# bacon205/Multimodal_eeg_fmri

Measured on AMD Instinct MI355X. Metric: pairs_per_sec_per_node, higher is better.
Workload: dtype bf16

## Files before the change

### multimodal_eeg_fmri_amd/csrc/attention.hip

```cpp
#include "common.h"

namespace {

constexpr int VR = 32;

__device__ __forceinline__ bf16x8 tr_frag32(const bf16* tile, int row0, int lane) {
    const int li = lane & 15, g = lane >> 4;
    const bf16* p = tile + (row0 + 8 * (g >> 1) + (li >> 2)) * VR + (g & 1) * 16 + 4 * (li & 3);
    typedef __attribute__((address_space(3))) s16x4 lds_s16x4;
    union { s16x4 s[2]; bf16x8 v; } u;
    u.s[0] = __builtin_amdgcn_ds_read_tr16_b64_v4i16((lds_s16x4*)(p));
    u.s[1] = __builtin_amdgcn_ds_read_tr16_b64_v4i16((lds_s16x4*)(p + 4 * VR));
    return u.v;
}

__device__ __forceinline__ int vperm(int key) {
    return (key & ~12) | ((key & 4) << 1) | ((key & 8) >> 1);
}

__device__ __forceinline__ uint32_t attn_block_hash(uint32_t seed, int bh, int q, int key, int L) {
    const uint32_t Lh = ((uint32_t)L + 1u) >> 1;
    uint32_t x = (((uint32_t)bh * Lh + ((uint32_t)q >> 1)) * Lh + ((uint32_t)key >> 1)) * 0x9E3779B1u + seed;
    x ^= x >> 13;
    x = __umul24(x, 0xB5297Bu);
    x ^= x >> 15;
    return x;
}
template <bool ALONG_KEYS>
__device__ __forceinline__ void attn_keep2(uint32_t seed, int bh, int mine, int other, int L, uint32_t thresh8, bool& k0, bool& k1) {
    if (ALONG_KEYS) {
        const uint32_t x = attn_block_hash(seed, bh, mine, other, L) >> (16 * (mine & 1));
        k0 = (x & 0xFFu) >= thresh8;
        k1 = ((x >> 8) & 0xFFu) >= thresh8;
    } else {
        const uint32_t x = attn_block_hash(seed, bh, other, mine, L) >> (8 * (mine & 1));
        k0 = (x & 0xFFu) >= thresh8;
        k1 = ((x >> 16) & 0xFFu) >= thresh8;
    }
}

__device__ __forceinline__ float xhalf_max(float v) {
    const auto r = __builtin_amdgcn_permlane32_swap(__float_as_uint(v), __float_as_uint(v), false, false);
    return fmaxf(__uint_as_float(r[0]), __uint_as_float(r[1]));
}
__device__ __forceinline__ float xhalf_sum(float v) {
    const auto r = __builtin_amdgcn_permlane32_swap(__float_as_uint(v), __float_as_uint(v), false, false);
    return __uint_as_float(r[0]) + __uint_as_float(r[1]);
}

__device__ __forceinline__ float fast_exp2(float x) { return __builtin_amdgcn_exp2f(x); }

__device__ __forceinline__ void zero8(bf16x8& v) {
#pragma unroll
    for (int j = 0; j < 8; ++j) v[j] = (bf16)0.f;
}

constexpr int KCH = 128;
constexpr int QCH = 128;

template <int DHP>
struct Hd {
    static_assert(DHP == 32 || DHP == 64, "padded head width");
    static constexpr int NS = DHP / 16;
    static constexpr int NT = DHP / 32;
    static constexpr int KS = DHP + 8;
    static constexpr int NG = DHP / 8;
    static __device__ __forceinline__ int tr_off(int rows, int row, int sg) { return (sg >> 2) * rows * VR + row * VR + (sg & 3) * 8; }
};

template <int DHP, bool EXACT>
struct Dims {
    int L, H, dh_;
    Dims(int L, int H, int dh) : L(L), H(H), dh_(dh) {}
    __device__ int dh() const { return dh_; }
};
template <int DHP>
struct Dims<DHP, true> {
    int L, H;
    Dims(int L, int H, int) : L(L), H(H) {}
    __device__ constexpr int dh() const { return DHP; }
};

template <int DHP, bool EXACT, bool DROP, bool FULL, bool MASK>
__global__ __launch_bounds__(256) void attn_fwd_kernel(const bf16* __restrict__ qkv, bf16* __restrict__ out,
                                                       float* __restrict__ lse, const Dims<DHP, EXACT> dm, float scale_log2,
                                                       uint32_t dthresh, uint32_t dseed, float dinv,
                                                       const uint32_t* epoch, const float* __restrict__ amask, size_t amask_bh) {
    using T = Hd<DHP>;
    constexpr int NS = T::NS, NT = T::NT, KS = T::KS, NG = T::NG;
    const int L = dm.L, H = dm.H, dh = dm.dh();
    dseed = mm_eff_seed(dseed, epoch);
    if (MASK) amask += (size_t)(blockIdx.z * H + blockIdx.y) * amask_bh;
    __shared__ __attribute__((aligned(16))) bf16 Ks[KCH * KS];
    __shared__ __attribute__((aligned(16))) bf16 Vs[NT * KCH * VR];
    const int E = H * dh, E3 = 3 * E;
    const int b = blockIdx.z, h = blockIdx.y;
    const int tid = threadIdx.x, lane = tid & 63, wave = tid >> 6;
    const int lr = lane & 31, lh = lane >> 5;
    const int q = blockIdx.x * 128 + wave * 32 + lr;
    const bf16* base = qkv + (size_t)b * L * E3 + h * dh;

    bf16x8 qf[NS];
#pragma unroll
    for (int s = 0; s < NS; ++s) {
        zero8(qf[s]);
        if (q < L && 16 * s + 8 * lh < dh) qf[s] = *reinterpret_cast<const bf16x8*>(base + (size_t)q * E3 + 16 * s + 8 * lh);
    }
    f32x16 o[NT];
#pragma unroll
    for (int t = 0; t < NT; ++t)
#pragma unroll
        for (int r = 0; r < 16; ++r) o[t][r] = 0.f;
    float m_run = -INFINITY, l_run = 0.f;

    constexpr int NI = KCH * NG / 256;
    uint4 kreg[NI], vreg[NI];
    auto load_chunk = [&](int k0) __attribute__((always_inline)) {
        const int kn = min(KCH, L - k0);
#pragma unroll
        for (int i = 0; i < NI; ++i) {
            const int s = tid + i * 256, key = s / NG, sg = s % NG;
            kreg[i] = make_uint4(0, 0, 0, 0); vreg[i] = make_uint4(0, 0, 0, 0);
            if (key < kn && sg * 8 < dh) {
                const bf16* row = base + (size_t)(k0 + key) * E3;
                kreg[i] = *reinterpret_cast<const uint4*>(row + E + sg * 8);
                vreg[i] = *reinterpret_cast<const uint4*>(row + 2 * E + sg * 8);
            }
        }
    };
    load_chunk(0);
#pragma unroll
    for (int s = 0; s < NS; ++s) asm volatile("" : : "v"(qf[s]));
    for (int k0 = 0; k0 < L; k0 += KCH) {
        const int kn = min(KCH, L - k0);
        const int kn32 = (kn + 31) & ~31;
        __syncthreads();
#pragma unroll
        for (int i = 0; i < NI; ++i) {
            const int s = tid + i * 256, key = s / NG, sg = s % NG;
            if (key >= kn32) continue;
            *reinterpret_cast<uint4*>(Ks + key * KS + sg * 8) = kreg[i];
            *reinterpret_cast<uint4*>(Vs + T::tr_off(KCH, vperm(key), sg)) = vreg[i];
        }
        __syncthreads();
        if (k0 + KCH < L) load_chunk(k0 + KCH);
        bf16x8 kfr[NS];
#pragma unroll
        for (int s = 0; s < NS; ++s) kfr[s] = *reinterpret_cast<const bf16x8*>(Ks + lr * KS + 16 * s + 8 * lh);
        for (int kt = 0; kt < kn32; kt += 32) {
            f32x16 sacc;
#pragma unroll
            for (int r = 0; r < 16; ++r) sacc[r] = 0.f;
#pragma unroll
            for (int s = 0; s < NS; ++s) sacc = __builtin_amdgcn_mfma_f32_32x32x16_bf16(kfr[s], qf[s], sacc, 0, 0, 0);
            bf16x8 vfr[NT][2];
#pragma unroll
            for (int t = 0; t < NT; ++t)
#pragma unroll
                for (int s = 0; s < 2; ++s) vfr[t][s] = tr_frag32(Vs + t * KCH * VR, kt + 16 * s, lane);
            if (kt + 32 < kn32)
#pragma unroll
                for (int s = 0; s < NS; ++s) kfr[s] = *reinterpret_cast<const bf16x8*>(Ks + (kt + 32 + lr) * KS + 16 * s + 8 * lh);
            const float sc2 = MASK ? 1.f : scale_log2;
            float mx = -INFINITY;
#pragma unroll
            for (int r = 0; r < 16; ++r) {
                const int key = kt + (r & 3) + 8 * (r >> 2) + 4 * lh;
                float sc = sacc[r];
                if (MASK) {
                    sc *= scale_log2;
                    if (key < kn) sc += amask[(size_t)min(q, L - 1) * L + k0 + key] * 1.4426950408889634f;
                }
                sacc[r] = (FULL || key < kn) ? sc : -INFINITY;
                mx = fmaxf(mx, sacc[r]);
            }
            mx = xhalf_max(mx);
            if (__builtin_amdgcn_ballot_w64(mx * sc2 > m_run + 8.f)) {
                const float m_new = fmaxf(m_run, mx * sc2);
                const float alpha = fast_exp2(m_run - ((MASK && m_new == -INFINITY) ? 0.f : m_new));
                l_run *= alpha;
                m_run = m_new;
#pragma unroll
                for (int t = 0; t < NT; ++t)
#pragma unroll
                    for (int r = 0; r < 16; ++r) o[t][r] *= alpha;
            }
            const float m_neg = (MASK && m_run == -INFINITY) ? 0.f : -m_run;
            float ps = 0.f;
            union { bf16x8 v[2]; bf16x2 h[8]; } pu;
#pragma unroll
            for (int r = 0; r < 16; r += 2) {
                float p0 = fast_exp2(fmaf(sacc[r], sc2, m_neg)), p1 = fast_exp2(fmaf(sacc[r + 1], sc2, m_neg));
                ps += p0;
                ps += p1;
                if (DROP) {
                    bool kp0, kp1;
                    attn_keep2<true>(dseed, b * H + h, q, k0 + kt + (r & 3) + 8 * (r >> 2) + 4 * lh, L, dthresh, kp0, kp1);
                    p0 = kp0 ? p0 : 0.f; p1 = kp1 ? p1 : 0.f;
                }
                typedef __attribute__((ext_vector_type(2))) float f32x2_t;
                pu.h[r >> 1] = __builtin_convertvector((f32x2_t){p0, p1}, bf16x2);
            }
            l_run += ps;
#pragma unroll
            for (int t = 0; t < NT; ++t)
#pragma unroll
                for (int s = 0; s < 2; ++s) o[t] = __builtin_amdgcn_mfma_f32_32x32x16_bf16(vfr[t][s], pu.v[s], o[t], 0, 0, 0);
        }
    }
    const float l_tot = xhalf_sum(l_run);
    const float inv = (DROP ? dinv : 1.f) / l_tot;
    if (q < L) {
        bf16* orow = out + ((size_t)b * L + q) * E + h * dh;
#pragma unroll
        for (int t = 0; t < NT; ++t)
#pragma unroll
            for (int g = 0; g < 4; ++g) {
                const int d = 32 * t + 8 * g + 4 * lh;
                if (d >= dh) continue;
                bf16x4 v = {(bf16)(o[t][4 * g] * inv), (bf16)(o[t][4 * g + 1] * inv), (bf16)(o[t][4 * g + 2] * inv), (bf16)(o[t][4 * g + 3] * inv)};
                *reinterpret_cast<bf16x4*>(orow + d) = v;
            }
        if (lse && lh == 0) lse[((size_t)b * H + h) * L + q] = (m_run + log2f(l_tot)) * 0.6931471805599453f;
    }
}

template <int DHP, bool EXACT, bool DROP, bool FULL, bool MASK>
__global__ __launch_bounds__(256) void attn_bwd_dq_kernel(const bf16* __restrict__ qkv, const bf16* __restrict__ out,
                                                          const bf16* __restrict__ dout, const float* __restrict__ lse,
                                                          bf16* __restrict__ dqkv, float* __restrict__ delta,
                                                          const Dims<DHP, EXACT> dm, float scale, uint32_t dthresh,
                                                          uint32_t dseed, float dinv, const uint32_t* epoch,
                                                          const float* __restrict__ amask, size_t amask_bh) {
    using T = Hd<DHP>;
    constexpr int NS = T::NS, NT = T::NT, KS = T::KS, NG = T::NG;
    const int L = dm.L, H = dm.H, dh = dm.dh();
    dseed = mm_eff_seed(dseed, epoch);
    if (MASK) amask += (size_t)(blockIdx.z * H + blockIdx.y) * amask_bh;
    __shared__ __attribute__((aligned(16))) bf16 Ks[KCH * KS];
    __shared__ __attribute__((aligned(16))) bf16 Vs[KCH * KS];
    __shared__ __attribute__((aligned(16))) bf16 Kr[NT * KCH * VR];
    const int E = H * dh, E3 = 3 * E;
    const int b = blockIdx.z, h = blockIdx.y;
    const int tid = threadIdx.x, lane = tid & 63, wave = tid >> 6;
    const int lr = lane & 31, lh = lane >> 5;
    const int q = blockIdx.x * 128 + wave * 32 + lr;
    const bool qok = q < L;
    const bf16* base = qkv + (size_t)b * L * E3 + h * dh;
    const float scale_log2 = scale * 1.4426950408889634f;

    bf16x8 qf[NS], dof[NS];
    float dl = 0.f;
#pragma unroll
    for (int s = 0; s < NS; ++s) {
        zero8(qf[s]); zero8(dof[s]);
        if (qok && 16 * s + 8 * lh < dh) {
            qf[s] = *reinterpret_cast<const bf16x8*>(base + (size_t)q * E3 + 16 * s + 8 * lh);
            const size_t oi = ((size_t)b * L + q) * E + h * dh + 16 * s + 8 * lh;
            dof[s] = *reinterpret_cast<const bf16x8*>(dout + oi);
            const bf16x8 of = *reinterpret_cast<const bf16x8*>(out + oi);
#pragma unroll
            for (int j = 0; j < 8; ++j) dl += (float)dof[s][j] * (float)of[j];
        }
    }
    dl = xhalf_sum(dl);
    const float lse2 = qok ? lse[((size_t)b * H + h) * L + q] * 1.4426950408889634f : 0.f;
    if (qok && lh == 0) delta[((size_t)b * H + h) * L + q] = dl;

    f32x16 dq[NT];
#pragma unroll
    for (int t = 0; t < NT; ++t)
#pragma unroll
        for (int r = 0; r < 16; ++r) dq[t][r] = 0.f;

    constexpr int NI = KCH * NG / 256;
    uint4 kreg[NI], vreg[NI];
    auto load_chunk = [&](int k0) __attribute__((always_inline)) {
        const int kn = min(KCH, L - k0);
#pragma unroll
        for (int i = 0; i < NI; ++i) {
            const int s = tid + i * 256, key = s / NG, sg = s % NG;
            kreg[i] = make_uint4(0, 0, 0, 0); vreg[i] = make_uint4(0, 0, 0, 0);
            if (key < kn && sg * 8 < dh) {
                const bf16* row = base + (size_t)(k0 + key) * E3;
                kreg[i] = *reinterpret_cast<const uint4*>(row + E + sg * 8);
                vreg[i] = *reinterpret_cast<const uint4*>(row + 2 * E + sg * 8);
            }
        }
    };
    load_chunk(0);
#pragma unroll
    for (int s = 0; s < NS; ++s) asm volatile("" : : "v"(qf[s]), "v"(dof[s]));
    asm volatile("" : : "v"(dl), "v"(lse2));
    for (int k0 = 0; k0 < L; k0 += KCH) {
        const int kn = min(KCH, L - k0);
        const int kn32 = (kn + 31) & ~31;
        __syncthreads();
#pragma unroll
        for (int i = 0; i < NI; ++i) {
            const int s = tid + i * 256, key = s / NG, sg = s % NG;
            if (key >= kn32) continue;
            *reinterpret_cast<uint4*>(Ks + key * KS + sg * 8) = kreg[i];
            *reinterpret_cast<uint4*>(Vs + key * KS + sg * 8) = vreg[i];
            *reinterpret_cast<uint4*>(Kr + T::tr_off(KCH, vperm(key), sg)) = kreg[i];
        }
        __syncthreads();
        if (k0 + KCH < L) load_chunk(k0 + KCH);
        for (int kt = 0; kt < kn32; kt += 32) {
            f32x16 sacc, dp;
#pragma unroll
            for (int r = 0; r < 16; ++r) { sacc[r] = 0.f; dp[r] = 0.f; }
            bf16x8 kfr[NS], vfr[NS];
#pragma unroll
            for (int s = 0; s < NS; ++s) {
                kfr[s] = *reinterpret_cast<const bf16x8*>(Ks + (kt + lr) * KS + 16 * s + 8 * lh);
                vfr[s] = *reinterpret_cast<const bf16x8*>(Vs + (kt + lr) * KS + 16 * s + 8 * lh);
            }
#pragma unroll
            for (int s = 0; s < NS; ++s) {
                sacc = __builtin_amdgcn_mfma_f32_32x32x16_bf16(kfr[s], qf[s], sacc, 0, 0, 0);
                dp = __builtin_amdgcn_mfma_f32_32x32x16_bf16(vfr[s], dof[s], dp, 0, 0, 0);
            }
            bf16x8 ktfr[NT][2];
#pragma unroll
            for (int t = 0; t < NT; ++t)
#pragma unroll
                for (int s = 0; s < 2; ++s) ktfr[t][s] = tr_frag32(Kr + t * KCH * VR, kt + 16 * s, lane);
            bf16x8 dsf[2];
            bool kp[16];
            if (DROP)
#pragma unroll
                for (int r = 0; r < 16; r += 2)
                    attn_keep2<true>(dseed, b * H + h, q, k0 + kt + (r & 3) + 8 * (r >> 2) + 4 * lh, L, dthresh, kp[r], kp[r + 1]);
#pragma unroll
            for (int r = 0; r < 16; ++r) {
                const int key = kt + (r & 3) + 8 * (r >> 2) + 4 * lh;
                float sc = fmaf(sacc[r], scale_log2, -lse2);
                if (MASK && key < kn) sc += amask[(size_t)min(q, L - 1) * L + k0 + key] * 1.4426950408889634f;
                const float p = (FULL || key < kn) ? fast_exp2(sc) : 0.f;
                float dpr = dp[r];
                if (DROP) dpr = fmaf(kp[r] ? dpr : 0.f, dinv, -dl);
                else dpr -= dl;
                dsf[r >> 3][r & 7] = (bf16)(p * dpr);
            }
#pragma unroll
            for (int t = 0; t < NT; ++t)
#pragma unroll
                for (int s = 0; s < 2; ++s) dq[t] = __builtin_amdgcn_mfma_f32_32x32x16_bf16(ktfr[t][s], dsf[s], dq[t], 0, 0, 0);
        }
    }
    if (qok) {
        bf16* drow = dqkv + ((size_t)b * L + q) * E3 + h * dh;
#pragma unroll
        for (int t = 0; t < NT; ++t)
#pragma unroll
            for (int g = 0; g < 4; ++g) {
                const int d = 32 * t + 8 * g + 4 * lh;
                if (d >= dh) continue;
                bf16x4 v = {(bf16)(dq[t][4 * g] * scale), (bf16)(dq[t][4 * g + 1] * scale), (bf16)(dq[t][4 * g + 2] * scale), (bf16)(dq[t][4 * g + 3] * scale)};
                *reinterpret_cast<bf16x4*>(drow + d) = v;
            }
    }
}

template <int DHP, bool EXACT, bool DROP, bool FULL, bool MASK>
__global__ __launch_bounds__(256) void attn_bwd_dkv_kernel(const bf16* __restrict__ qkv, const bf16* __restrict__ dout,
                                                           const float* __restrict__ lse, const float* __restrict__ delta,
                                                           bf16* __restrict__ dqkv, const Dims<DHP, EXACT> dm, float scale,
                                                           uint32_t dthresh, uint32_t dseed, float dinv,
                                                           const uint32_t* epoch, const float* __restrict__ amask, size_t amask_bh) {
    using T = Hd<DHP>;
    constexpr int NS = T::NS, NT = T::NT, KS = T::KS, NG = T::NG;
    const int L = dm.L, H = dm.H, dh = dm.dh();
    dseed = mm_eff_seed(dseed, epoch);
    if (MASK) amask += (size_t)(blockIdx.z * H + blockIdx.y) * amask_bh;
    __shared__ __attribute__((aligned(16))) bf16 Qs[QCH * KS];
    __shared__ __attribute__((aligned(16))) bf16 Ds[QCH * KS];
    __shared__ __attribute__((aligned(16))) bf16 Qr[NT * QCH * VR];
    __shared__ __attribute__((aligned(16))) bf16 Dr[NT * QCH * VR];
    __shared__ float Ls[QCH], Dl[QCH];
    const int E = H * dh, E3 = 3 * E;
    const int b = blockIdx.z, h = blockIdx.y;
    const int tid = threadIdx.x, lane = tid & 63, wave = tid >> 6;
    const int lr = lane & 31, lh = lane >> 5;
    const int key = blockIdx.x * 128 + wave * 32 + lr;
    const bool kok = key < L;
    const bf16* base = qkv + (size_t)b * L * E3 + h * dh;
    const float scale_log2 = scale * 1.4426950408889634f;

    bf16x8 kf[NS], vf[NS];
#pragma unroll
    for (int s = 0; s < NS; ++s) {
        zero8(kf[s]); zero8(vf[s]);
        if (kok && 16 * s + 8 * lh < dh) {
            kf[s] = *reinterpret_cast<const bf16x8*>(base + (size_t)key * E3 + E + 16 * s + 8 * lh);
            vf[s] = *reinterpret_cast<const bf16x8*>(base + (size_t)key * E3 + 2 * E + 16 * s + 8 * lh);
        }
    }
    f32x16 dk[NT], dv[NT];
#pragma unroll
    for (int t = 0; t < NT; ++t)
#pragma unroll
        for (int r = 0; r < 16; ++r) { dk[t][r] = 0.f; dv[t][r] = 0.f; }

    constexpr int NI = QCH * NG / 256;
    static_assert(QCH <= 256, "one lse / delta value per thread");
    uint4 qreg[NI], dreg[NI];
    float lreg = INFINITY, dlreg = 0.f;
    auto load_chunk = [&](int q0) __attribute__((always_inline)) {
        const int qn = min(QCH, L - q0);
#pragma unroll
        for (int i = 0; i < NI; ++i) {
            const int s = tid + i * 256, qi = s / NG, sg = s % NG;
            qreg[i] = make_uint4(0, 0, 0, 0); dreg[i] = make_uint4(0, 0, 0, 0);
            if (qi < qn && sg * 8 < dh) {
                qreg[i] = *reinterpret_cast<const uint4*>(base + (size_t)(q0 + qi) * E3 + sg * 8);
                dreg[i] = *reinterpret_cast<const uint4*>(dout + ((size_t)b * L + q0 + qi) * E + h * dh + sg * 8);
            }
        }
        const bool ok = tid < qn;
        lreg = ok ? lse[((size_t)b * H + h) * L + q0 + tid] : INFINITY;
        dlreg = ok ? delta[((size_t)b * H + h) * L + q0 + tid] : 0.f;
    };
    load_chunk(0);
#pragma unroll
    for (int s = 0; s < NS; ++s) asm volatile("" : : "v"(kf[s]), "v"(vf[s]));
    for (int q0 = 0; q0 < L; q0 += QCH) {
        const int qn = min(QCH, L - q0);
        const int qn32 = (qn + 31) & ~31;
        __syncthreads();
#pragma unroll
        for (int i = 0; i < NI; ++i) {
            const int s = tid + i * 256, qi = s / NG, sg = s % NG;
            if (qi >= qn32) continue;
            *reinterpret_cast<uint4*>(Qs + qi * KS + sg * 8) = qreg[i];
            *reinterpret_cast<uint4*>(Ds + qi * KS + sg * 8) = dreg[i];
            *reinterpret_cast<uint4*>(Qr + T::tr_off(QCH, vperm(qi), sg)) = qreg[i];
            *reinterpret_cast<uint4*>(Dr + T::tr_off(QCH, vperm(qi), sg)) = dreg[i];
        }
        if (tid < qn32) { Ls[tid] = lreg * 1.4426950408889634f; Dl[tid] = dlreg; }
        __syncthreads();
        if (q0 + QCH < L) load_chunk(q0 + QCH);
        for (int qt = 0; qt < qn32; qt += 32) {
            f32x16 sacc, dp;
#pragma unroll
            for (int r = 0; r < 16; ++r) { sacc[r] = 0.f; dp[r] = 0.f; }
            bf16x8 qar[NS], dar[NS];
#pragma unroll
            for (int s = 0; s < NS; ++s) {
                qar[s] = *reinterpret_cast<const bf16x8*>(Qs + (qt + lr) * KS + 16 * s + 8 * lh);
                dar[s] = *reinterpret_cast<const bf16x8*>(Ds + (qt + lr) * KS + 16 * s + 8 * lh);
            }
#pragma unroll
            for (int s = 0; s < NS; ++s) {
                sacc = __builtin_amdgcn_mfma_f32_32x32x16_bf16(qar[s], kf[s], sacc, 0, 0, 0);
                dp = __builtin_amdgcn_mfma_f32_32x32x16_bf16(dar[s], vf[s], dp, 0, 0, 0);
            }
            bf16x8 dtar[NT][2], qtar[NT][2];
#pragma unroll
            for (int t = 0; t < NT; ++t)
#pragma unroll
                for (int s = 0; s < 2; ++s) {
                    dtar[t][s] = tr_frag32(Dr + t * QCH * VR, qt + 16 * s, lane);
                    qtar[t][s] = tr_frag32(Qr + t * QCH * VR, qt + 16 * s, lane);
                }
            bf16x8 pf[2], dsf[2];
            bool kp[16];
            if (DROP)
#pragma unroll
                for (int r = 0; r < 16; r += 2)
                    attn_keep2<false>(dseed, b * H + h, key, q0 + qt + (r & 3) + 8 * (r >> 2) + 4 * lh, L, dthresh, kp[r], kp[r + 1]);
#pragma unroll
            for (int r = 0; r < 16; ++r) {
                const int qi = qt + (r & 3) + 8 * (r >> 2) + 4 * lh;
                float sc = fmaf(sacc[r], scale_log2, -Ls[qi]);
                if (MASK && kok && qi < qn) sc += amask[(size_t)(q0 + qi) * L + key] * 1.4426950408889634f;
                const float p = (FULL || kok) ? fast_exp2(sc) : 0.f;
                pf[r >> 3][r & 7] = (bf16)((!DROP || kp[r]) ? p : 0.f);
                const float u = DROP ? fmaf(kp[r] ? dp[r] : 0.f, dinv, -Dl[qi]) : dp[r] - Dl[qi];
                dsf[r >> 3][r & 7] = (bf16)(p * u);
            }
#pragma unroll
            for (int t = 0; t < NT; ++t)
#pragma unroll
                for (int s = 0; s < 2; ++s) {
                    dv[t] = __builtin_amdgcn_mfma_f32_32x32x16_bf16(dtar[t][s], pf[s], dv[t], 0, 0, 0);
                    dk[t] = __builtin_amdgcn_mfma_f32_32x32x16_bf16(qtar[t][s], dsf[s], dk[t], 0, 0, 0);
                }
        }
    }
    if (kok) {
        bf16* krow = dqkv + ((size_t)b * L + key) * E3 + E + h * dh;
        bf16* vrow = krow + E;
        const float dvs = DROP ? dinv : 1.f;
#pragma unroll
        for (int t = 0; t < NT; ++t)
#pragma unroll
            for (int g = 0; g < 4; ++g) {
                const int d = 32 * t + 8 * g + 4 * lh;
                if (d >= dh) continue;
                bf16x4 a = {(bf16)(dk[t][4 * g] * scale), (bf16)(dk[t][4 * g + 1] * scale), (bf16)(dk[t][4 * g + 2] * scale), (bf16)(dk[t][4 * g + 3] * scale)};
                bf16x4 c = {(bf16)(dv[t][4 * g] * dvs), (bf16)(dv[t][4 * g + 1] * dvs), (bf16)(dv[t][4 * g + 2] * dvs), (bf16)(dv[t][4 * g + 3] * dvs)};
                *reinterpret_cast<bf16x4*>(krow + d) = a;
                *reinterpret_cast<bf16x4*>(vrow + d) = c;
            }
    }
}

uint32_t attn_thresh(float p) { return p > 0.f ? (uint32_t)((double)p * 256.0 + 0.5) : 0u; }
float attn_keep_scale(uint32_t t) { return t ? 256.f / (256.f - (float)t) : 1.f; }

bool hd_supported(int dh) { return dh >= 16 && dh <= 64 && dh % 8 == 0; }

template <int DHP, bool EXACT>
void launch_fwd(const void* qkv, void* out, float* lse, int B, int L, int H, int dh, float scale, float drop_p,
                uint32_t seed, const uint32_t* seed_epoch, const float* attn_mask, int per_head, hipStream_t st) {
    const uint32_t dth = attn_thresh(drop_p);
    const size_t mask_bh = attn_mask && per_head ? (size_t)L * L : 0;
    const bool full = L % KCH == 0;
    auto kern = dth ? (full ? attn_fwd_kernel<DHP, EXACT, true, true, false> : attn_fwd_kernel<DHP, EXACT, true, false, false>)
                    : (full ? attn_fwd_kernel<DHP, EXACT, false, true, false> : attn_fwd_kernel<DHP, EXACT, false, false, false>);
    if (attn_mask) kern = dth ? attn_fwd_kernel<DHP, EXACT, true, false, true> : attn_fwd_kernel<DHP, EXACT, false, false, true>;
    hipLaunchKernelGGL(kern, dim3(ceil_div(L, 128), H, B), dim3(256), 0, st, (const bf16*)qkv, (bf16*)out, lse,
                       Dims<DHP, EXACT>(L, H, dh), scale * 1.4426950408889634f, dth, seed, attn_keep_scale(dth), seed_epoch,
                       attn_mask, mask_bh);
}

template <int DHP, bool EXACT>
int launch_bwd(const void* qkv, const void* out, const void* dout, const float* lse, void* dqkv, float* delta_ws,
               int B, int L, int H, int dh, float scale, float drop_p, uint32_t seed, const uint32_t* seed_epoch,
               const float* attn_mask, int per_head, hipStream_t st) {
    const uint32_t dth = attn_thresh(drop_p);
    const float dinv = attn_keep_scale(dth);
    const size_t mask_bh = attn_mask && per_head ? (size_t)L * L : 0;
    const bool full = L % KCH == 0 && L % QCH == 0;
    auto kdq = dth ? (full ? attn_bwd_dq_kernel<DHP, EXACT, true, true, false> : attn_bwd_dq_kernel<DHP, EXACT, true, false, false>)
                   : (full ? attn_bwd_dq_kernel<DHP, EXACT, false, true, false> : attn_bwd_dq_kernel<DHP, EXACT, false, false, false>);
    auto kdkv = dth ? (full ? attn_bwd_dkv_kernel<DHP, EXACT, true, true, false> : attn_bwd_dkv_kernel<DHP, EXACT, true, false, false>)
                    : (full ? attn_bwd_dkv_kernel<DHP, EXACT, false, true, false> : attn_bwd_dkv_kernel<DHP, EXACT, false, false, false>);
    if (attn_mask) {
        kdq = dth ? attn_bwd_dq_kernel<DHP, EXACT, true, false, true> : attn_bwd_dq_kernel<DHP, EXACT, false, false, true>;
        kdkv = dth ? attn_bwd_dkv_kernel<DHP, EXACT, true, false, true> : attn_bwd_dkv_kernel<DHP, EXACT, false, false, true>;
    }
    const dim3 grid(ceil_div(L, 128), H, B);
    const Dims<DHP, EXACT> dm(L, H, dh);
    hipLaunchKernelGGL(kdq, grid, dim3(256), 0, st, (const bf16*)qkv, (const bf16*)out, (const bf16*)dout, lse,
                       (bf16*)dqkv, delta_ws, dm, scale, dth, seed, dinv, seed_epoch, attn_mask, mask_bh);
    int rc = mm_check_launch(EXACT ? "attn_bwd_dq" : "attn_bwd_hd_dq");
    if (rc) return rc;
    hipLaunchKernelGGL(kdkv, grid, dim3(256), 0, st, (const bf16*)qkv, (const bf16*)dout, lse, delta_ws, (bf16*)dqkv,
                       dm, scale, dth, seed, dinv, seed_epoch, attn_mask, mask_bh);
    return mm_check_launch(EXACT ? "attn_bwd_dkv" : "attn_bwd_hd_dkv");
}

}

extern "C" {

int mm_attn_fwd(const void* qkv, void* out, float* lse, int B, int L, int H, int head_dim, float scale,
                float drop_p, uint32_t seed, const uint32_t* seed_epoch, const float* attn_mask, int attn_mask_per_head,
                hipStream_t st) {
    MM_REQUIRE(drop_p >= 0.f && drop_p < 1.f, "attn_fwd: drop_p");
    MM_REQUIRE(qkv && out && B > 0 && L > 0 && H > 0, "attn_fwd: null/invalid");
    MM_REQUIRE(head_dim == 32, "attn_fwd: head_dim=%d (kernel is specialised for 32)", head_dim);
    launch_fwd<32, true>(qkv, out, lse, B, L, H, head_dim, scale, drop_p, seed, seed_epoch, attn_mask, attn_mask_per_head, st);
    return mm_check_launch("attn_fwd");
}

int mm_attn_bwd(const void* qkv, const void* out, const void* dout, const float* lse, void* dqkv, float* delta_ws,
                int B, int L, int H, int head_dim, float scale, float drop_p, uint32_t seed,
                const uint32_t* seed_epoch, const float* attn_mask, int attn_mask_per_head, hipStream_t st) {
    MM_REQUIRE(qkv && out && dout && lse && dqkv && delta_ws && B > 0 && L > 0 && H > 0, "attn_bwd: null/invalid");
    MM_REQUIRE(head_dim == 32, "attn_bwd: head_dim=%d (kernel is specialised for 32)", head_dim);
    return launch_bwd<32, true>(qkv, out, dout, lse, dqkv, delta_ws, B, L, H, head_dim, scale, drop_p, seed, seed_epoch,
                                attn_mask, attn_mask_per_head, st);
}

int mm_attn_fwd_hd(const void* qkv, void* out, float* lse, int B, int L, int H, int head_dim, float scale,
                   float drop_p, uint32_t seed, const uint32_t* seed_epoch, const float* attn_mask, int attn_mask_per_head,
                   hipStream_t st) {
    MM_REQUIRE(hd_supported(head_dim), "attn_fwd_hd: head_dim=%d (supported: multiples of 8 in [16, 64])", head_dim);
    MM_REQUIRE(drop_p >= 0.f && drop_p < 1.f, "attn_fwd_hd: drop_p");
    MM_REQUIRE(qkv && out && B > 0 && L > 0 && H > 0, "attn_fwd_hd: null/invalid");
    auto launch = head_dim <= 32 ? launch_fwd<32, false> : launch_fwd<64, false>;
    launch(qkv, out, lse, B, L, H, head_dim, scale, drop_p, seed, seed_epoch, attn_mask, attn_mask_per_head, st);
    return mm_check_launch("attn_fwd_hd");
}

int mm_attn_bwd_hd(const void* qkv, const void* out, const void* dout, const float* lse, void* dqkv, float* delta_ws,
                   int B, int L, int H, int head_dim, float scale, float drop_p, uint32_t seed,
                   const uint32_t* seed_epoch, const float* attn_mask, int attn_mask_per_head, hipStream_t st) {
    MM_REQUIRE(hd_supported(head_dim), "attn_bwd_hd: head_dim=%d (supported: multiples of 8 in [16, 64])", head_dim);
    MM_REQUIRE(drop_p >= 0.f && drop_p < 1.f, "attn_bwd_hd: drop_p");
    MM_REQUIRE(qkv && out && dout && lse && dqkv && delta_ws && B > 0 && L > 0 && H > 0, "attn_bwd_hd: null/invalid");
    auto launch = head_dim <= 32 ? launch_bwd<32, false> : launch_bwd<64, false>;
    return launch(qkv, out, dout, lse, dqkv, delta_ws, B, L, H, head_dim, scale, drop_p, seed, seed_epoch, attn_mask,
                  attn_mask_per_head, st);
}

}
```

Measured before the change: 41560.

## Add fused single-block attention backward kernel for short sequences with head dim 32

Result: slower. 40740 (-2.0%).

```diff
diff --git a/multimodal_eeg_fmri_amd/csrc/attention.hip b/multimodal_eeg_fmri_amd/csrc/attention.hip
--- a/multimodal_eeg_fmri_amd/csrc/attention.hip
+++ b/multimodal_eeg_fmri_amd/csrc/attention.hip
@@ -4,13 +4,14 @@
 
 constexpr int VR = 32;
 
+template <int RS = VR>
 __device__ __forceinline__ bf16x8 tr_frag32(const bf16* tile, int row0, int lane) {
     const int li = lane & 15, g = lane >> 4;
-    const bf16* p = tile + (row0 + 8 * (g >> 1) + (li >> 2)) * VR + (g & 1) * 16 + 4 * (li & 3);
+    const bf16* p = tile + (row0 + 8 * (g >> 1) + (li >> 2)) * RS + (g & 1) * 16 + 4 * (li & 3);
     typedef __attribute__((address_space(3))) s16x4 lds_s16x4;
     union { s16x4 s[2]; bf16x8 v; } u;
     u.s[0] = __builtin_amdgcn_ds_read_tr16_b64_v4i16((lds_s16x4*)(p));
-    u.s[1] = __builtin_amdgcn_ds_read_tr16_b64_v4i16((lds_s16x4*)(p + 4 * VR));
+    u.s[1] = __builtin_amdgcn_ds_read_tr16_b64_v4i16((lds_s16x4*)(p + 4 * RS));
     return u.v;
 }
 
@@ -507,6 +508,203 @@
     }
 }
 
+constexpr int FUSED_LMAX = 512;
+constexpr int FDS = 36;
+constexpr int FPS = 36;
+
+template <bool DROP>
+__global__ __launch_bounds__(512) void attn_bwd_fused_kernel(const bf16* __restrict__ qkv, const bf16* __restrict__ out,
+                                                             const bf16* __restrict__ dout, const float* __restrict__ lse,
+                                                             bf16* __restrict__ dqkv, float* __restrict__ delta,
+                                                             const Dims<32, true> dm, float scale, uint32_t dthresh,
+                                                             uint32_t dseed, float dinv, const uint32_t* epoch) {
+    using T = Hd<32>;
+    constexpr int NS = T::NS, KS = T::KS;
+    const int L = dm.L, H = dm.H;
+    dseed = mm_eff_seed(dseed, epoch);
+    __shared__ __attribute__((aligned(16))) bf16 Qs[QCH * KS];
+    __shared__ __attribute__((aligned(16))) bf16 Ds[QCH * KS];
+    __shared__ __attribute__((aligned(16))) bf16 Qr[QCH * VR];
+    __shared__ __attribute__((aligned(16))) bf16 Dr[QCH * VR];
+    __shared__ __attribute__((aligned(16))) bf16 Kr[FUSED_LMAX * VR];
+    __shared__ __attribute__((aligned(16))) bf16 dSt[8 * 32 * FDS];
+    __shared__ __attribute__((aligned(16))) float Pq[2 * 8 * 32 * FPS];
+    __shared__ float Ls[QCH], Dl[QCH];
+    const int E = H * 32, E3 = 3 * E;
+    const int b = blockIdx.z, h = blockIdx.y, bh = b * H + h;
+    const int tid = threadIdx.x, lane = tid & 63, wave = tid >> 6;
+    const int lr = lane & 31, lh = lane >> 5;
+    const bf16* base = qkv + (size_t)b * L * E3 + h * 32;
+    const float scale_log2 = scale * 1.4426950408889634f;
+    const int nw = min(8, L / 32);
+    const bool act[2] = {wave * 32 < L, (wave + 8) * 32 < L};
+
+    bf16x8 kf[2][NS], vf[2][NS];
+    f32x16 dk[2], dv[2];
+#pragma unroll
+    for (int j = 0; j < 2; ++j) {
+        const int key = (wave + 8 * j) * 32 + lr;
+#pragma unroll
+        for (int s = 0; s < NS; ++s) {
+            zero8(kf[j][s]); zero8(vf[j][s]);
+            if (act[j]) {
+                kf[j][s] = *reinterpret_cast<const bf16x8*>(base + (size_t)key * E3 + E + 16 * s + 8 * lh);
+                vf[j][s] = *reinterpret_cast<const bf16x8*>(base + (size_t)key * E3 + 2 * E + 16 * s + 8 * lh);
+            }
+        }
+#pragma unroll
+        for (int r = 0; r < 16; ++r) { dk[j][r] = 0.f; dv[j][r] = 0.f; }
+    }
+    for (int s = tid; s < L * 4; s += 512) {
+        const int key = s >> 2, sg = s & 3;
+        *reinterpret_cast<uint4*>(Kr + key * VR + sg * 8) = *reinterpret_cast<const uint4*>(base + (size_t)key * E3 + E + sg * 8);
+    }
+
+    const bool is_d = wave < 4;
+    const int qi = (tid & 255) >> 1, cg = tid & 1;
+    uint4 areg[2], oreg[2];
+    float lreg = 0.f;
+    auto load_chunk = [&](int q0) __attribute__((always_inline)) {
+        const size_t orow = ((size_t)b * L + q0 + qi) * E + h * 32;
+        const bf16* src = is_d ? dout + orow : base + (size_t)(q0 + qi) * E3;
+#pragma unroll
+        for (int i = 0; i < 2; ++i) {
+            areg[i] = *reinterpret_cast<const uint4*>(src + (cg + 2 * i) * 8);
+            if (is_d) oreg[i] = *reinterpret_cast<const uint4*>(out + orow + (cg + 2 * i) * 8);
+        }
+        if (!is_d && cg == 0) lreg = lse[(size_t)bh * L + q0 + qi];
+    };
+    load_chunk(0);
+#pragma unroll
+    for (int j = 0; j < 2; ++j)
+#pragma unroll
+        for (int s = 0; s < NS; ++s) asm volatile("" : : "v"(kf[j][s]), "v"(vf[j][s]));
+    bf16* const myds = dSt + wave * 32 * FDS;
+    for (int q0 = 0; q0 < L; q0 += QCH) {
+        __syncthreads();
+        {
+            bf16* rows = (is_d ? Ds : Qs) + qi * KS;
+            bf16* rowt = (is_d ? Dr : Qr) + vperm(qi) * VR;
+#pragma unroll
+            for (int i = 0; i < 2; ++i) {
+                *reinterpret_cast<uint4*>(rows + (cg + 2 * i) * 8) = areg[i];
+                *reinterpret_cast<uint4*>(rowt + (cg + 2 * i) * 8) = areg[i];
+            }
+            if (is_d) {
+                float dl = 0.f;
+#pragma unroll
+                for (int i = 0; i < 2; ++i) {
+                    union { uint4 u; bf16x8 v; } dd, oo;
+                    dd.u = areg[i]; oo.u = oreg[i];
+#pragma unroll
+                    for (int j = 0; j < 8; ++j) dl += (float)dd.v[j] * (float)oo.v[j];
+                }
+                dl += __shfl_xor(dl, 1);
+                if (cg == 0) { Dl[qi] = dl; delta[(size_t)bh * L + q0 + qi] = dl; }
+            } else if (cg == 0) {
+                Ls[qi] = lreg * 1.4426950408889634f;
+            }
+        }
+        __syncthreads();
+        if (q0 + QCH < L) load_chunk(q0 + QCH);
+        for (int qt = 0; qt < QCH; qt += 32) {
+            float* const pq = Pq + (((q0 + qt) >> 5) & 1) * (8 * 32 * FPS);
+            if (act[0]) {
+                bf16x8 qar[NS], dar[NS], dtar[2], qtar[2];
+#pragma unroll
+                for (int s = 0; s < NS; ++s) {
+                    qar[s] = *reinterpret_cast<const bf16x8*>(Qs + (qt + lr) * KS + 16 * s + 8 * lh);
+                    dar[s] = *reinterpret_cast<const bf16x8*>(Ds + (qt + lr) * KS + 16 * s + 8 * lh);
+                }
+#pragma unroll
+                for (int s = 0; s < 2; ++s) {
+                    dtar[s] = tr_frag32(Dr, qt + 16 * s, lane);
+                    qtar[s] = tr_frag32(Qr, qt + 16 * s, lane);
+                }
+                f32x16 dqa;
+#pragma unroll
+                for (int r = 0; r < 16; ++r) dqa[r] = 0.f;
+#pragma unroll
+                for (int j = 0; j < 2; ++j) {
+                    if (!act[j]) continue;
+                    const int kb = (wave + 8 * j) * 32, key = kb + lr;
+                    f32x16 sacc, dp;
+#pragma unroll
+                    for (int r = 0; r < 16; ++r) { sacc[r] = 0.f; dp[r] = 0.f; }
+#pragma unroll
+                    for (int s = 0; s < NS; ++s) {
+                        sacc = __builtin_amdgcn_mfma_f32_32x32x16_bf16(qar[s], kf[j][s], sacc, 0, 0, 0);
+                        dp = __builtin_amdgcn_mfma_f32_32x32x16_bf16(dar[s], vf[j][s], dp, 0, 0, 0);
+                    }
+                    bf16x8 pf[2];
+                    union { bf16x8 v[2]; bf16x4 q[4]; } ds;
+                    bool kp[16];
+                    if (DROP)
+#pragma unroll
+                        for (int r = 0; r < 16; r += 2)
+                            attn_keep2<false>(dseed, bh, key, q0 + qt + (r & 3) + 8 * (r >> 2) + 4 * lh, L, dthresh, kp[r], kp[r + 1]);
+#pragma unroll
+                    for (int r = 0; r < 16; ++r) {
+                        const int qq = qt + (r & 3) + 8 * (r >> 2) + 4 * lh;
+                        const float p = fast_exp2(fmaf(sacc[r], scale_log2, -Ls[qq]));
+                        pf[r >> 3][r & 7] = (bf16)((!DROP || kp[r]) ? p : 0.f);
+                        const float u = DROP ? fmaf(kp[r] ? dp[r] : 0.f, dinv, -Dl[qq]) : dp[r] - Dl[qq];
+                        ds.v[r >> 3][r & 7] = (bf16)(p * u);
+                    }
+#pragma unroll
+                    for (int s = 0; s < 2; ++s) {
+                        dv[j] = __builtin_amdgcn_mfma_f32_32x32x16_bf16(dtar[s], pf[s], dv[j], 0, 0, 0);
+                        dk[j] = __builtin_amdgcn_mfma_f32_32x32x16_bf16(qtar[s], ds.v[s], dk[j], 0, 0, 0);
+                    }
+#pragma unroll
+                    for (int g = 0; g < 4; ++g) *reinterpret_cast<bf16x4*>(myds + lr * FDS + 8 * g + 4 * lh) = ds.q[g];
+                    __builtin_amdgcn_fence(__ATOMIC_RELEASE, "wavefront");
+                    __builtin_amdgcn_wave_barrier();
+                    __builtin_amdgcn_fence(__ATOMIC_ACQUIRE, "wavefront");
+#pragma unroll
+                    for (int s = 0; s < 2; ++s) {
+                        const bf16x8 ktr = tr_frag32(Kr, kb + 16 * s, lane), dst = tr_frag32<FDS>(myds, 16 * s, lane);
+                        dqa = __builtin_amdgcn_mfma_f32_32x32x16_bf16(ktr, dst, dqa, 0, 0, 0);
+                    }
+                    __builtin_amdgcn_fence(__ATOMIC_RELEASE, "wavefront");
+                    __builtin_amdgcn_wave_barrier();
+                    __builtin_amdgcn_fence(__ATOMIC_ACQUIRE, "wavefront");
+                }
+                float* prow = pq + (wave * 32 + lr) * FPS + 4 * lh;
+#pragma unroll
+                for (int g = 0; g < 4; ++g)
+                    *reinterpret_cast<float4*>(prow + 8 * g) = make_float4(dqa[4 * g], dqa[4 * g + 1], dqa[4 * g + 2], dqa[4 * g + 3]);
+            }
+            __syncthreads();
+            {
+                const float* pr = pq + (tid >> 4) * FPS + 2 * (tid & 15);
+                float s0 = 0.f, s1 = 0.f;
+                for (int w = 0; w < nw; ++w) {
+                    const float2 v = *reinterpret_cast<const float2*>(pr + w * 32 * FPS);
+                    s0 += v.x; s1 += v.y;
+                }
+                const bf16x2 v = {(bf16)(s0 * scale), (bf16)(s1 * scale)};
+                *reinterpret_cast<bf16x2*>(dqkv + ((size_t)b * L + q0 + qt + (tid >> 4)) * E3 + h * 32 + 2 * (tid & 15)) = v;
+            }
+        }
+    }
+    const float dvs = DROP ? dinv : 1.f;
+#pragma unroll
+    for (int j = 0; j < 2; ++j) {
+        if (!act[j]) continue;
+        bf16* krow = dqkv + ((size_t)b * L + (wave + 8 * j) * 32 + lr) * E3 + E + h * 32;
+        bf16* vrow = krow + E;
+#pragma unroll
+        for (int g = 0; g < 4; ++g) {
+            const int d = 8 * g + 4 * lh;
+            bf16x4 a = {(bf16)(dk[j][4 * g] * scale), (bf16)(dk[j][4 * g + 1] * scale), (bf16)(dk[j][4 * g + 2] * scale), (bf16)(dk[j][4 * g + 3] * scale)};
+            bf16x4 c = {(bf16)(dv[j][4 * g] * dvs), (bf16)(dv[j][4 * g + 1] * dvs), (bf16)(dv[j][4 * g + 2] * dvs), (bf16)(dv[j][4 * g + 3] * dvs)};
+            *reinterpret_cast<bf16x4*>(krow + d) = a;
+            *reinterpret_cast<bf16x4*>(vrow + d) = c;
+        }
+    }
+}
+
 uint32_t attn_thresh(float p) { return p > 0.f ? (uint32_t)((double)p * 256.0 + 0.5) : 0u; }
 float attn_keep_scale(uint32_t t) { return t ? 256.f / (256.f - (float)t) : 1.f; }
 
@@ -533,6 +731,14 @@
     const uint32_t dth = attn_thresh(drop_p);
     const float dinv = attn_keep_scale(dth);
     const size_t mask_bh = attn_mask && per_head ? (size_t)L * L : 0;
+    if constexpr (DHP == 32 && EXACT) {
+        if (!attn_mask && L % QCH == 0 && L <= FUSED_LMAX) {
+            hipLaunchKernelGGL(dth ? attn_bwd_fused_kernel<true> : attn_bwd_fused_kernel<false>, dim3(1, H, B), dim3(512), 0,
+                               st, (const bf16*)qkv, (const bf16*)out, (const bf16*)dout, lse, (bf16*)dqkv, delta_ws,
+                               Dims<32, true>(L, H, dh), scale, dth, seed, dinv, seed_epoch);
+            return mm_check_launch("attn_bwd_fused");
+        }
+    }
     const bool full = L % KCH == 0 && L % QCH == 0;
     auto kdq = dth ? (full ? attn_bwd_dq_kernel<DHP, EXACT, true, true, false> : attn_bwd_dq_kernel<DHP, EXACT, true, false, false>)
                    : (full ? attn_bwd_dq_kernel<DHP, EXACT, false, true, false> : attn_bwd_dq_kernel<DHP, EXACT, false, false, false>);
```
